# flexcompute/tidy3d

Measured on AMD Instinct MI355X. Metric: Mcells/s on 512^3 Yee grid, higher is better.
Workload: dtype f32; 1 GPU; v0: vacuum, PEC walls, curl stencil only; 512^3 Yee cells, Ez point dipole (GaussianPulse 200 THz), random +-1e-3 initial fields; parallelism=z-slab x1, bytes_per_cell_step=72

## Files before the change

### tidy3d_amd/csrc/fdtd_capi.hip

```cpp
#include <hip/hip_runtime.h>
#include <rccl/rccl.h>

#include <array>
#include <cmath>
#include <cstdarg>
#include <cstdio>
#include <cstdlib>
#include <cstring>
#include <deque>
#include <map>
#include <string>
#include <utility>
#include <algorithm>
#include <vector>

#include "../../include/fdtd_hip.h"
#include "fdtd_kernels.hpp"
#include "fdtd_fused2.hpp"
#include "fdtd_strip.hpp"
#include "fdtd_shell2_host.hpp"
#include "fdtd_aniso.hpp"

using namespace fdtd;

// ... 154 lines not shown
  std::vector<TileClasses> tile_cls;
  int tile_split = -1;
  float2* lut = nullptr;
  int n_media = 0;
  float ca1 = 1.f, cb1 = 0.f;
  std::vector<float> cb_host;
  PmlAxisDev pml[3];
  float *damp_fb[3] = {}, *damp_fc[3] = {};
  int damp_lo[3] = {0, 0, 0}, damp_hi[3] = {0, 0, 0};
  bool has_damp = false;
  std::vector<AdeGroup> ade;
  Disp disp;
  SrcPaged spg;
  std::map<std::array<int, 6>, int> box_paged;
  int spg_on = -1;
  int whatif = 0;
  int disp_on = -1;
  std::vector<AnisoGroup> aniso;
  std::vector<PointSrc> psrc;
  std::vector<Tfsf> tfsf;
  std::vector<Monitor> mons;
  hipStream_t stream = nullptr, comm_stream = nullptr;
  hipEvent_t ev0 = nullptr, ev1 = nullptr;
  std::vector<hipEvent_t> kev;
  std::vector<int> kev_kind;
  double* energy_dev = nullptr;
  int decay_every = 0;
  double shutoff = 0.0;
  long long decay_ref = 0;
  double energy_max = 0.0;
// ... 857 lines not shown
  const MatP mp = mat_params(h);
  DispP dp{nullptr, nullptr, nullptr};
  if (use_disp) dp = DispP{h->disp.dseg, h->disp.cs, h->disp.e1};
  const bool damp = !clip && h->has_damp;
  SrcP sr_used = sr;
  if (h->whatif == 9 && !sr.sseg && !damp && (!use_disp || clip)) {
    SrcPaged& S = h->spg;
    const size_t nseg = (size_t)g.nz * g.ny * ((g.nx + 255) / 256);
    if (!S.sseg && S.state != 1) {
      S.sseg_host.assign(nseg, -1);
      SrcT tab{};
      if (dev_upload(h, &S.sseg, (const int*)S.sseg_host.data(), nseg) || dev_upload(h, &S.tab, &tab, 1)) return -1;
    }
    if (S.sseg && S.state != 1) { sr_used.sseg = S.sseg; sr_used.t = S.tab; }
  }
  const int wv = h->whatif == 19 ? 9 : ((h->whatif >= 1 && h->whatif <= 15 && h->whatif != 9) ? h->whatif : 0);
  const auto word = [&](bool rep) {
    return fused2_opt(h->mem_hints != 0, h->mat4 != nullptr, !(tb->mons.empty() && (!tb->with_sources || h->src_h_nodes == 0) && !tb->dstart),
                      clip != nullptr, damp, use_disp, sr_used.sseg != nullptr, wv, rep, W);
  };
  const bool rep_capable = n_seams > 0 && !clip && (W == 16 || h->seam_defer == 2) && fused2_rep_word(word(false));
  const int opt = word(rep_capable && (h->seam_pending || h->whatif == 17));
  const auto no_sweep = [&] { return fail(h, "launch_fused2: no instantiation of the sweep for opt 0x%x, %d waves", opt, W); };
  if (!fused2_instantiated(fused2_lb(W, opt), opt)) return no_sweep();
  if (sr.sseg) { *sources2_done = true; h->spg.pairs++; }
  float* const rep_arr = h->seam_buf ? h->seam_buf + seam_scratch_floats(g, nbx) : nullptr;
  if (h->seam_pending && !rep_capable) flush_seams(h, st);
  h->seam_pending = false;
  bool defer = defer_ok && rep_capable && h->seam_defer != 0 && h->whatif == 0;
  if (defer) {
    bool e_post = false;
    for (const PointSrc& s : h->psrc) e_post = e_post || (s.n_e && n + 1 < s.n_steps);
    if ((e_post && !*sources2_done) || (h->has_damp && !dmp.e2)) defer = false;
  }
  const int blocks = remap ? ((total + 7) / 8) * 8 : total;
  const FdtdSolver::TileClasses* tc = tile_classes(h, W, zc, box, nbx, nby, nbz, use_disp, sr_used.sseg != nullptr);
  const bool split = tc && (use_disp || sr_used.sseg || (tc->n_bg > 0 && (h->tile_split == 1 || 8 * tc->n_bg >= tc->n_all)));
  const bool launched = launch_fused2_step(Fused2Launch{st, W, opt, blocks, g, h->f, h->f2, sp, mp, zc, nbx, nby, nbz, remap, inj, h->seam_buf, dmp, box,
                                                        TileClassP{split ? tc->dev : nullptr}, dp, sr_used});
  time_end(h, st);
  if (!launched) return no_sweep();
// ... 3080 lines not shown
      h->twostep_w = w;
      h->twostep_zc = zc;
      return 0;
    }
    case FDTD_OPT_PML_SPLIT: h->pml_split = value < 0 ? -1 : (value != 0); return 0;
    case FDTD_OPT_SHELL_PAIRS: h->shell_on = value < 0 ? -1 : value; return 0;
    case FDTD_OPT_STRIP: if (value % 64 < 1 || (value / 64 != 3 && value / 64 != 4)) break; h->strip_zc = value % 64; h->strip_occ = value / 64; return 0;
    case FDTD_OPT_SHELL2: h->shell2_on = value < 0 ? -1 : (value > 3 ? 1 : value); return 0;
    case FDTD_OPT_DEBUG_SYNC: h->debug_sync = value != 0; return 0;
    case FDTD_OPT_TILE_SPLIT: h->tile_split = value < 0 ? -1 : (value != 0); return 0;
    case FDTD_OPT_SRC_PAGED:
      h->spg_on = value < 0 ? -1 : (value != 0);
      if (h->spg.state == -1 && value != 0) h->spg.state = 0;
      return 0;
    case FDTD_OPT_SLAB_BOXES_FIRST: if (value < 0 || value > 3) break; h->slab_boxes_first = value; return 0;
    case FDTD_OPT_WHATIF: if (value < 0 || value > 19) break; h->whatif = value; return 0;
    case FDTD_OPT_SEAM_DEFER: if (value > 2) break; h->seam_defer = value < 0 ? -1 : value; return 0;
    case FDTD_OPT_DISP:
      if (h->disp.state == 1 && value == 0) break;
      h->disp_on = value < 0 ? -1 : (value != 0);
      if (h->disp.state == -1 && value != 0) h->disp.state = 0;
      return 0;
    case FDTD_OPT_SHELL2_SHAPE: {
      if (value <= 0) { h->shell2_qw = 0; h->shell2_ww = 8; h->shell2_zcw = 0; h->shell2_ws = 6; h->shell2_zcs = 0; return 0; }
      const int qw = value % 128, ww = (value >> 7) % 8 + ((value >> 7) % 8 == 0 ? 8 : 0), zcw = (value >> 10) % 128;
      const int ws = (value >> 17) % 16, zcs = (value >> 21) % 128;
      if ((qw != 0 && qw < 3) || qw > 64 || ws > 8) break;
      h->shell2_qw = qw; h->shell2_ww = ww; h->shell2_zcw = zcw;
      h->shell2_ws = ws > 0 ? ws : 6; h->shell2_zcs = zcs;
      return 0;
    }
// ... 45 lines not shown
```

### tidy3d_amd/csrc/fdtd_fused2.hip

```cpp
#include "fdtd_static_kernels.hpp"
#include "fdtd_kernels2.hpp"

namespace fdtd {

void launch_inject_values(hipStream_t st, float* val, const float* w_re, const float* w_im, const float2* wave,
                          long long step, int n) {
  hipLaunchKernelGGL(inject_values_kernel, dim3(1), dim3(256), 0, st, val, w_re, w_im, wave, step, n);
}

static FDTD_F2_LAUNCHER(launch_fused2_step_base, FDTD_F2_LIST_OWN)

bool launch_fused2_step(const Fused2Launch& L) {
  if (L.opt & kF2Src) return launch_fused2_step_src(L);
  if (fused2_whatif(L.opt)) return launch_fused2_step_whatif(L);
  if (L.opt & kF2Disp) return launch_fused2_step_disp(L);
  if (L.opt & kF2Clip) return launch_fused2_step_clip(L);
  return launch_fused2_step_base(L);
}

void launch_inject_table(hipStream_t st, float* tab, long long stride, long long off, const float* w_re, const float* w_im,
                         const float2* wave, long long n_steps, int n) {
  const unsigned blocks = (unsigned)((n_steps * n + 255) / 256);
  hipLaunchKernelGGL(inject_table_kernel, dim3(blocks), dim3(256), 0, st, tab, stride, off, w_re, w_im, wave, n_steps, n);
}

void launch_pair_record(hipStream_t st, const PairRecP& r, long long max_cells, const GridP& g, const FieldP& a, const FieldP& b,
                        const float* cap) {
  const dim3 grid((unsigned)((max_cells + 255) / 256), (unsigned)(r.n_mon * 6));
  hipLaunchKernelGGL(pair_record_kernel, grid, dim3(256), 0, st, r, g, a, b, cap);
}

void launch_dft_record_dump(hipStream_t st, const DftDumpP& r, const float* dump, float2* acc, long long cells, long long fstride,
                            const float2* phase, int nf) {
  const dim3 grid((unsigned)((cells + 255) / 256), (unsigned)r.n);
  hipLaunchKernelGGL(dft_record_dump_kernel, grid, dim3(256), 0, st, r, dump, acc, cells, fstride, phase, nf);
}

void launch_seams(hipStream_t st, const GridP& g, const FieldP& b, const StepP& s, const MatP& m, const float* seam,
                  int n_seams, const DampT& dmp, const ClipP& clip, const InjP& inj, const SrcP& sr, float* rep) {
  const long long nt = (long long)n_seams * (clip.j1 - clip.j0) * (clip.k1 - clip.k0);
  if (nt <= 0) return;
  const unsigned blocks = (unsigned)((nt + 255) / 256);
  hipLaunchKernelGGL(seam_kernel, dim3(blocks), dim3(256), 0, st, g, b, s, m, seam, n_seams, dmp, clip, inj, sr, rep);
}

void launch_seam_flush(hipStream_t st, const GridP& g, const FieldP& b, const float* rep, int n_seams) {
  const long long nt = (long long)n_seams * g.ny * g.nz;
  if (nt <= 0) return;
  hipLaunchKernelGGL(seam_flush_kernel, dim3((unsigned)((nt + 255) / 256)), dim3(256), 0, st, g, b, rep, n_seams);
}

}
```

### tidy3d_amd/csrc/fdtd_fused2.hpp

```cpp
#pragma once
#include "fdtd_kernels.hpp"

namespace fdtd {

constexpr int kMaxInj = 256;
struct InjP {
  int n;
  const int* start;
  const int4* ent;
  const float* val;
  const float* val2;
  int e2_in_sweep;
  float* cap;
  const int* dstart;
  const int* dlist;
  const struct DumpBox* dboxes;
  float* dump;
};
struct DumpBox {
  int lo0, lo1, lo2, nx, ny, nz;
  int off[6];
};
constexpr int kMaxDumps = 8;
struct DampT {
// ... 16 lines not shown
  const float* e1b;
  const float* h2b;
  const float* e2b;
};
struct SrcP {
  const int* sseg = nullptr;
  const SrcT* t = nullptr;
};
constexpr int kF2NT = 1;
constexpr int kF2Mat = 2;
constexpr int kF2Mon = 4;
constexpr int kF2Damp = 8;
constexpr int kF2Clip = 16;
constexpr int kF2Disp = 32;
constexpr int kF2Src = 64;
constexpr int kF2WhatifShift = 8, kF2WhatifMask = 15;
constexpr int kF2NoExj = 4096;
constexpr int kF2Rep = 8192;
constexpr int fused2_whatif(int opt) { return (opt >> kF2WhatifShift) & kF2WhatifMask; }
constexpr int fused2_whatif_word(int wv) { return kF2NT | (wv << kF2WhatifShift); }
constexpr bool fused2_rep_word(int opt) { return (opt & ~(kF2NT | kF2Mat | kF2Damp)) == 0; }

constexpr int fused2_opt(bool nt, bool mat, bool mon, bool clip, bool damp, bool disp, bool src, int whatif, bool rep, int W) {
  int opt = (nt ? kF2NT : 0) | (mat ? kF2Mat : 0) | (mon ? kF2Mon : 0) | (clip ? kF2Clip : (damp ? kF2Damp : 0)) |
            (disp ? kF2Disp | kF2NT : 0) | (src ? kF2Src | kF2Mon | kF2NT : 0);
  if (whatif && opt == kF2NT && (W == 16 || whatif == 13 || whatif == 14)) opt = fused2_whatif_word(whatif);
  return opt | (rep ? kF2Rep : 0);
}
constexpr int fused2_lb(int waves, int opt) {
  if ((opt & kF2Rep) || fused2_whatif(opt)) return 1024;
  if (waves <= 8) return 512;
  return (waves <= 12 && !(opt & (kF2Src | kF2Disp))) ? 768 : 1024;
// ... 9 lines not shown
#define FDTD_F2_LIST_REP(X) FDTD_F2_ANY_MAT(FDTD_F2_AT1024, X, kF2Rep) FDTD_F2_ANY_MAT(FDTD_F2_AT1024, X, kF2Rep | kF2Damp)
#define FDTD_F2_LIST_BASE(X) FDTD_F2_BASE_AT(FDTD_F2_AT512, X) FDTD_F2_BASE_AT(FDTD_F2_AT768, X) FDTD_F2_BASE_AT(FDTD_F2_AT1024, X)
#define FDTD_F2_LIST_CLIP(X) FDTD_F2_ANY_MON(FDTD_F2_AT512, X, kF2Clip) FDTD_F2_ANY_MON(FDTD_F2_AT768, X, kF2Clip) FDTD_F2_ANY_MON(FDTD_F2_AT1024, X, kF2Clip)
#define FDTD_F2_DISP_MON(AT, X, O) AT(X, kF2Disp | kF2Mat | kF2NT | (O)) AT(X, kF2Disp | kF2Mat | kF2NT | kF2Mon | (O))
#define FDTD_F2_DISP_AT(AT, X) FDTD_F2_DISP_MON(AT, X, 0) FDTD_F2_DISP_MON(AT, X, kF2Damp) FDTD_F2_DISP_MON(AT, X, kF2Clip)
#define FDTD_F2_LIST_DISP(X) FDTD_F2_DISP_AT(FDTD_F2_AT512, X) FDTD_F2_DISP_AT(FDTD_F2_AT1024, X)
#define FDTD_F2_SRC_MAT(AT, X, O) AT(X, kF2Src | kF2Mon | kF2NT | (O)) AT(X, kF2Src | kF2Mon | kF2NT | kF2Mat | (O))
#define FDTD_F2_SRC_DISP(AT, X, O) AT(X, kF2Src | kF2Mon | kF2NT | kF2Mat | kF2Disp | (O))
#define FDTD_F2_SRC_AT(AT, X)                                                                          \
  FDTD_F2_SRC_MAT(AT, X, 0) FDTD_F2_SRC_MAT(AT, X, kF2Damp) FDTD_F2_SRC_MAT(AT, X, kF2Clip)              \
  FDTD_F2_SRC_DISP(AT, X, kF2Clip) FDTD_F2_SRC_DISP(AT, X, 0) FDTD_F2_SRC_DISP(AT, X, kF2Damp)
#define FDTD_F2_LIST_SRC(X) FDTD_F2_SRC_AT(FDTD_F2_AT512, X) FDTD_F2_SRC_AT(FDTD_F2_AT1024, X)
#define FDTD_F2_WV(X, WV) X(1024, fused2_whatif_word(WV))
#define FDTD_F2_LIST_WHATIF(X)                                                                                        \
  FDTD_F2_WV(X, 1) FDTD_F2_WV(X, 2) FDTD_F2_WV(X, 3) FDTD_F2_WV(X, 4) FDTD_F2_WV(X, 5) FDTD_F2_WV(X, 6) FDTD_F2_WV(X, 7) FDTD_F2_WV(X, 8) \
  FDTD_F2_WV(X, 9) FDTD_F2_WV(X, 10) FDTD_F2_WV(X, 11) FDTD_F2_WV(X, 12) FDTD_F2_WV(X, 13) FDTD_F2_WV(X, 14) FDTD_F2_WV(X, 15)
#define FDTD_F2_LIST_OWN(X) FDTD_F2_LIST_REP(X) FDTD_F2_LIST_BASE(X)
#define FDTD_F2_LIST_ALL(X) FDTD_F2_LIST_OWN(X) FDTD_F2_LIST_CLIP(X) FDTD_F2_LIST_DISP(X) FDTD_F2_LIST_SRC(X) FDTD_F2_LIST_WHATIF(X)
constexpr int fused2_key(int lb, int opt) { return opt * 2048 + lb; }
constexpr bool fused2_instantiated(int lb, int opt) {
  switch (fused2_key(lb, opt)) {
#define FDTD_F2_X(LBV, OV) case fused2_key(LBV, OV):
    FDTD_F2_LIST_ALL(FDTD_F2_X)
#undef FDTD_F2_X
      return true;
    default: return false;
  }
}
constexpr bool fused2_words_instantiated() {
  for (int W = 4; W <= 16; ++W)
    for (int in = 0; in < 128; ++in) {
      const bool nt = in & 1, mat = in & 2, mon = in & 4, clip = in & 8, damp = in & 16, disp = in & 32, src = in & 64;
      if ((clip && damp) || (disp && !mat)) continue;
      for (int wv = 0; wv <= 15; ++wv) {
        const int opt = fused2_opt(nt, mat, mon, clip, damp, disp, src, wv, false, W);
        if (wv && !fused2_whatif(opt)) continue;
        if (!fused2_instantiated(fused2_lb(W, opt), opt)) return false;
        const int rep = fused2_opt(nt, mat, mon, clip, damp, disp, src, wv, true, W);
        if (!clip && fused2_rep_word(opt) && !fused2_instantiated(fused2_lb(W, rep), rep)) return false;
      }
    }
  return true;
}
static_assert(fused2_words_instantiated(), "fused2_opt forms a word that no list of instantiations holds");

#if !defined(FDTD_NO_EXJ)
#define FDTD_NO_EXJ 0
#endif
constexpr bool fused2_exj(int lb, int opt) { return !FDTD_NO_EXJ && (opt & kF2Damp) == 0 && !(lb == 512 && (opt & kF2Mat) != 0); }
constexpr int fused2_xch_arrays(int lb, int opt) {
  const int wv = fused2_whatif(opt);
  if (wv) return wv == 13 ? 9 : ((wv >= 10 && wv <= 12) ? 6 + (wv == 11 ? 2 : 3) : 8);
  return fused2_exj(lb, opt) ? 9 : 8;
}
constexpr size_t fused2_lds_bytes(int lb, int opt, int waves) {
  return ((size_t)fused2_xch_arrays(lb, opt) * waves * 64 + ((opt & kF2Damp) ? 2 * 64 : 0)) * sizeof(float4) + ((opt & kF2Mat) ? (size_t)kMaxMedia * sizeof(float2) : 0);
}
static_assert(fused2_lds_bytes(1024, kF2NT | kF2Mat | kF2Mon | kF2Clip | kF2Disp | kF2Src, 16) <= 160 * 1024 && fused2_lds_bytes(1024, kF2Mat | kF2Damp, 16) <= 160 * 1024 &&
              2 * fused2_lds_bytes(512, kF2NT, 8) <= 160 * 1024 && 2 * fused2_lds_bytes(512, kF2Mat | kF2Damp, 8) <= 160 * 1024,
              "fused2_step_kernel: LDS of a workgroup (two per CU for eight waves)");
constexpr bool fused2_lds_pinned(int lb, int opt) {
  const int wv = fused2_whatif(opt), w = lb / 64;
  if (wv) return fused2_lds_bytes(lb, opt, 16) == ((size_t)(wv == 13 ? 9 : ((wv >= 10 && wv <= 12) ? 6 + (wv == 11 ? 2 : 3) : 8)) * 16 * 64) * sizeof(float4);
  return fused2_lds_bytes(lb, opt, w) == ((size_t)(fused2_exj(lb, opt) ? 9 : 8) * w * 64 + ((opt & 8) ? 2 * 64 : 0)) * sizeof(float4) + ((opt & 2) ? (size_t)kMaxMedia * sizeof(float2) : 0);
}
#define FDTD_F2_X(LBV, OV) && fused2_lds_pinned(LBV, OV)
static_assert(true FDTD_F2_LIST_ALL(FDTD_F2_X), "fused2_lds_bytes: the LDS of a listed instantiation changed");
#undef FDTD_F2_X
constexpr int kMaxCap = 1024;
constexpr int kSeamArrays = 13;

void launch_inject_values(hipStream_t st, float* val, const float* w_re, const float* w_im, const float2* wave,
                          long long step, int n);
struct Fused2Launch {
  hipStream_t st;
  int waves, opt, grid_blocks;
  GridP g; FieldP a, b; StepP s; MatP m;
  int zchunk, nbx, nby, nbz, xcd_remap;
  InjP inj; float* seam; DampT dmp; ClipP clip; TileClassP tcl; DispP dp; SrcP sr;
// ... 22 lines not shown
  BoxP box[kPairMons];
  int nc[kPairMons];
  int comp[kPairMons][6];
  int cap_off[kPairMons];
  float* out_n[kPairMons];
  float* out_m[kPairMons];
};
void launch_pair_record(hipStream_t st, const PairRecP& r, long long max_cells, const GridP& g, const FieldP& a, const FieldP& b,
                        const float* cap);
struct DftDumpP { int n; int slot[3]; int off[3]; };
void launch_dft_record_dump(hipStream_t st, const DftDumpP& r, const float* dump, float2* acc, long long cells, long long fstride,
                            const float2* phase, int nf);
void launch_seams(hipStream_t st, const GridP& g, const FieldP& b, const StepP& s, const MatP& m, const float* seam,
                  int n_seams, const DampT& dmp, const ClipP& clip, const InjP& inj, const SrcP& sr = SrcP{}, float* rep = nullptr);
constexpr int kRepArraysHost = 7;
inline size_t seam_scratch_floats(const GridP& g, int n_tiles_x) { return (size_t)n_tiles_x * kSeamArrays * (size_t)(g.nz + 2) * (size_t)g.ny; }
inline size_t seam_rep_floats(const GridP& g, int n_tiles_x) { return (size_t)n_tiles_x * kRepArraysHost * (size_t)g.nz * (size_t)g.ny; }
void launch_seam_flush(hipStream_t st, const GridP& g, const FieldP& b, const float* rep, int n_seams);

}
```

### tidy3d_amd/csrc/fdtd_kernels2.hpp

```cpp
#pragma once
#include "fdtd_fused2.hpp"

namespace fdtd {

__global__ __launch_bounds__(256) void pair_record_kernel(PairRecP r, GridP g, FieldP a, FieldP b, const float* cap) {
  const int mi = blockIdx.y / 6, ic = blockIdx.y % 6;
  if (mi >= r.n_mon || ic >= r.nc[mi]) return;
  const BoxP bx = r.box[mi];
  const long long cells = (long long)bx.nx * bx.ny * bx.nz;
  const long long t = (long long)blockIdx.x * blockDim.x + threadIdx.x;
  if (t >= cells) return;
  const int c = r.comp[mi][ic];
  const int lx = (int)(t % bx.nx), ly = (int)((t / bx.nx) % bx.ny), lz = (int)(t / ((long long)bx.nx * bx.ny));
  const long long p = (long long)(bx.lo2 + lz) * g.sxy + (long long)(bx.lo1 + ly) * g.nx + bx.lo0 + lx;
  const long long idx = (long long)ic * cells + t;
  const float* fa = c == 0 ? a.ex : (c == 1 ? a.ey : (c == 2 ? a.ez : (c == 3 ? a.hx : (c == 4 ? a.hy : a.hz))));
  const float* fb = c == 0 ? b.ex : (c == 1 ? b.ey : (c == 2 ? b.ez : (c == 3 ? b.hx : (c == 4 ? b.hy : b.hz))));
  const float mid = cap[r.cap_off[mi] + idx];
  float* on = r.out_n[mi];
  float* om = r.out_m[mi];
  if (c < 3) {
    if (on && !r.pre_done) on[idx] = 1.0f * fa[p];
    if (om) om[idx] = 1.0f * mid;
  } else {
// ... 24 lines not shown
  if (g >= n_steps * n) return;
  const long long step = g / n;
  const int t = (int)(g % n);
  const float2 a = wave[step];
  tab[step * stride + off + t] = w_re[t] * a.x - w_im[t] * a.y;
}

__global__ __launch_bounds__(256) void inject_values_kernel(float* val, const float* w_re, const float* w_im,
                                                            const float2* wave, long long step, int n) {
  const int t = threadIdx.x;
  if (t >= n) return;
  const float2 a = wave[step];
  val[t] = w_re[t] * a.x - w_im[t] * a.y;
}

__device__ __forceinline__ long long seam_at(const GridP& g, int seam, int arr, int j, int k) {
  return (((long long)seam * kSeamArrays + arr) * (g.nz + 2) + (k + 1)) * g.ny + j;
}

constexpr int kRepArrays = 7;
__device__ __forceinline__ long long rep_base(const GridP& g, int n_tiles_x) {
  return (long long)n_tiles_x * kSeamArrays * (g.nz + 2) * g.ny;
}
__device__ __forceinline__ long long rep_at(const GridP& g, int seam, int arr, int j, int k) {
  return (((long long)seam * kRepArrays + arr) * g.nz + k) * g.ny + j;
}

__device__ __forceinline__ float lane_next(float v) {
#if defined(__HIP_DEVICE_COMPILE__)
  const int x = __builtin_bit_cast(int, v);
  return __builtin_bit_cast(float, __builtin_amdgcn_update_dpp(x, x, 0x130, 0xf, 0xf, false));
#else
  return __shfl_down(v, 1);
#endif
}
__device__ __forceinline__ float lane_prev(float v) {
#if defined(__HIP_DEVICE_COMPILE__)
// ... 20 lines not shown
#endif
}
__device__ __forceinline__ void lds_dma_fence() {
#if defined(__HIP_DEVICE_COMPILE__)
  asm volatile("s_waitcnt lgkmcnt(0)" ::: "memory");
#endif
}

__device__ __forceinline__ int opaque_lane(int v) {
#if defined(__HIP_DEVICE_COMPILE__)
  asm volatile("" : "+v"(v));
#endif
  return v;
}

__device__ __forceinline__ int lane_value(int v, int l) {
#if defined(__HIP_DEVICE_COMPILE__)
  return __builtin_amdgcn_readlane(v, l);
#else
  return __shfl(v, l);
#endif
}

template <int LB, int OPT>
__device__ __forceinline__ void fused2_step_tile(const GridP& g, const FieldP& a, const FieldP& b, const StepP& s, const MatP& m,
                                                 int zchunk, int nbx, int nby, int nbz, const InjP& inj,
                                                 float* __restrict__ seam, const DampT& dmp, const ClipP& clip, int t,
                                                 const DispP& dp, const SrcP& sr) {
  constexpr int V = 4;
  constexpr bool SRC = (OPT & kF2Src) != 0;
  constexpr bool NT = (OPT & kF2NT) != 0, MAT = (OPT & kF2Mat) != 0, MON = (OPT & kF2Mon) != 0;
  constexpr bool DISP = (OPT & kF2Disp) != 0;
  constexpr int WHATIF = fused2_whatif(OPT);
  constexpr int PF = (WHATIF >= 10 && WHATIF <= 12) ? WHATIF : 0;
  constexpr bool EZL = WHATIF == 15;
// ... 23 lines not shown
    for (int q = 0; q < NXCH; ++q) xch[q * slot + me] = z4;
  }
  [[maybe_unused]] float4* xdm = xch + (EXJ ? 9 : 8) * slot;
  [[maybe_unused]] float2* lut_s = reinterpret_cast<float2*>(xdm + (DAMP ? 2 * 64 : 0));
  if constexpr (MAT) {
    for (int q = me; q < m.n_media; q += slot) lut_s[q] = m.lut[q];
  }
  if constexpr (DAMP) {
    if (ty == 0) {
      const int ii = (tile_x * 64 + tx) * V;
      float4 b4 = {1.f, 1.f, 1.f, 1.f}, c4 = {1.f, 1.f, 1.f, 1.f};
      if (ii < g.nx) { b4 = *reinterpret_cast<const float4*>(dmp.fb[0] + ii); c4 = *reinterpret_cast<const float4*>(dmp.fc[0] + ii); }
      xdm[tx] = b4; xdm[64 + tx] = c4;
    }
  }
  __syncthreads();
  const float ca = m.ca1, cb = m.cb1;
  const int k0 = (CLIP ? clip.k0 : 0) + tile_z * zchunk;
  const int k1 = min(k0 + zchunk, CLIP ? clip.k1 : g.nz);
  const int kA = k0 > 0 ? k0 - 1 : 0;
  int j = (CLIP ? clip.j0 : 0) + tile_y * R + ty - 2;
  const bool row_ok = (j >= 0) && (j < g.ny);
  if (!row_ok) {
    if constexpr (WHATIF != 6 && WHATIF != 7 && WHATIF != 8)
      for (int k = kA; k <= k1; ++k) { __syncthreads(); if constexpr (WHATIF != 2) __syncthreads(); }
    return;
  }
  const int i0 = (tile_x * 64 + tx) * V;
  const unsigned ux = (unsigned)i0;
  const unsigned ub = ux * 4u;
// ... 82 lines not shown
      const float czp = dmp.fc[2][kA - 1];
      const float4 b4 = xdm[tx], c4 = xdm[64 + tx];
      const float bx[V] = {b4.x, b4.y, b4.z, b4.w}, cx[V] = {c4.x, c4.y, c4.z, c4.w};
#pragma unroll
      for (int e = 0; e < V; ++e) { ho[e] *= bx[e] * cyv * czp; hoy[e] *= cx[e] * byv * czp; }
    }
#pragma unroll
    for (int e = 0; e < V; ++e) h1x[e] = upd_h(ho[e], ch, ezj[e] - ezm[e], ipy, eyk[e] - eym[e], ipz);
#pragma unroll
    for (int e = 0; e < V; ++e) {
      const float ez_ip = (e + 1 < V) ? ezm[(e + 1) % V] : ezx;
      h1y[e] = upd_h(hoy[e], ch, exk[e] - exm[e], ipz, ez_ip - ezm[e], ipx[e]);
    }
  }
  int cur = 0;
  const long long seam_arr = (long long)(g.nz + 2) * g.ny;
  const long long seam_row = seam_at(g, tile_x, 0, j, 0);
  struct Ld {
    float exn[V], eyn[V], ezk[V], exj[V], ezj[V], hxn[V], hyn[V], hzn[V];
    float eyx_g, ezx_g;
    float exn_m, ez_mm, ey_mm, ex_jm, hy_o, hz_o;
  };
  [[maybe_unused]] float4* pfb = xch + NXCH * slot;
  [[maybe_unused]] auto pf_issue = [&](int k) __attribute__((always_inline)) {
    if constexpr (PF != 0) {
      const long long pb = (long long)k * g.sxy + rowb;
      const long long up = (k < g.nz) ? g.sxy : 0;
      lds_dma_fence();
      if constexpr (PF == 10) {
        lds_dma16(uni(a.hx + pb), ubc, pfb + 0 * slot + ty * 64, tx);
        lds_dma16(uni(a.hy + pb), ubc, pfb + 1 * slot + ty * 64, tx);
        lds_dma16(uni(a.hz + pb), ubc, pfb + 2 * slot + ty * 64, tx);
// ... 96 lines not shown
    if constexpr (PF != 0) {
      lds_dma_wait();
      if constexpr (PF == 10) { pf_take(0, L.hxn); pf_take(1, L.hyn); pf_take(2, L.hzn); }
      else if constexpr (PF == 11) { pf_take(0, L.eyn); pf_take(1, L.hyn); }
      else { pf_take(0, L.exn); pf_take(1, L.eyn); pf_take(2, L.ezk); }
    }
  };
  Ld LA, LB2;
  auto body = [&](int k, Ld& L) __attribute__((always_inline)) {
    const int txo = (MAT || DAMP) ? tx : opaque_lane(tx);
    const int i0o = (tile_x * 64 + txo) * V;
    const bool act = i0o < g.nx, last_x = i0o + V >= g.nx, first_x = i0o == 0;
    const bool xh = act && txo == 0 && (!first_x || per_x);
    [[maybe_unused]] const bool wall_x0 = first_x && !pmc_x0 && !per_x;
    const bool seam_l = (txo == 63 && !last_x) || (per_x && last_x), seam_r = txo == 0 && (tile_x > 0 || per_x);
    const long long seam_back = (tile_x > 0 ? -1 : (long long)(nbx - 1)) * kSeamArrays * seam_arr;
    const long long pb = (long long)k * g.sxy + rowb;
    const float ipz = s.ipz[k], idz = s.idz[k];
    [[maybe_unused]] float bzk = 1.f, czk = 1.f;
    if constexpr (DAMP) { bzk = dmp.fb[2][min(k, g.nz - 1)]; czk = dmp.fc[2][min(k, g.nz - 1)]; }
    int q0 = 0, q1 = 0;
    if (inj.n > 0) { q0 = inj.start[k]; q1 = inj.start[k + 1]; }
    [[maybe_unused]] int d0 = 0, d1 = 0;
    if constexpr (MON) { if (inj.dstart) { d0 = inj.dstart[k]; d1 = inj.dstart[k + 1]; } }
    float hy_m = 0.f, hz_m = 0.f;
    float (&exn)[V] = L.exn, (&eyn)[V] = L.eyn, (&ezk)[V] = L.ezk, (&exj)[V] = L.exj, (&ezj)[V] = L.ezj;
    float (&hxn)[V] = L.hxn, (&hyn)[V] = L.hyn, (&hzn)[V] = L.hzn;
    [[maybe_unused]] uint32_t rw = kBgWord;
    if constexpr (MAT) {
      if (do_e1) rw = m.roww[((long long)min(k, g.nz - 1) * g.ny + j) * nbx + tile_x];
    }
// ... 231 lines not shown
                for (int e = 0; e < V; ++e) {
                  const int lx = i0o + e - bx.lo0;
                  if (lx >= 0 && lx < bx.nx && act && (!CLIP || (i0o + e >= clip.i0 && i0o + e < clip.i1))) {
                    if (bx.off[0] >= 0) inj.dump[bx.off[0] + rowo + lx] = e1xn[e];
                    if (bx.off[1] >= 0) inj.dump[bx.off[1] + rowo + lx] = e1yn[e];
                    if (bx.off[2] >= 0) inj.dump[bx.off[2] + rowo + lx] = e1zn[e];
                    if (bx.off[3] >= 0) inj.dump[bx.off[3] + rowo + lx] = hxn[e];
                    if (bx.off[4] >= 0) inj.dump[bx.off[4] + rowo + lx] = hyn[e];
                    if (bx.off[5] >= 0) inj.dump[bx.off[5] + rowo + lx] = hzn[e];
                  }
                }
              }
            }
          }
        }
        if (WHATIF != 9 && (CLIP || (own && k >= k0 && k < k1)) && act) {
          float* sp = seam + seam_row + (long long)k * g.ny;
          if (seam_l) {
            sp[0] = hyn[V - 1];
            sp[seam_arr] = hzn[V - 1];
            sp[2 * seam_arr] = e1xn[V - 1];
            sp[3 * seam_arr] = e1yn[V - 1];
            sp[4 * seam_arr] = e1zn[V - 1];
          }
          if (seam_r) {
            sp[5 * seam_arr + seam_back] = e1yn[0];
            sp[6 * seam_arr + seam_back] = e1zn[0];
          }
        }
      }
    }
    float h2x[V], h2y[V], h2z[V];
    unspecified<V>(h2x); unspecified<V>(h2y); unspecified<V>(h2z);
    if (do_h2 && k > kA) {
      if constexpr (DAMP) {
        {
          const float4 b4 = xdm[tx];
          const float bx[V] = {b4.x, b4.y, b4.z, b4.w};
#pragma unroll
          for (int e = 0; e < V; ++e) h1x[e] *= bx[e] * cyv * cz_m;
        }
        {
// ... 47 lines not shown
        t0 = make_float4(e1x[0], e1x[1], e1x[2], e1x[3]); t1 = make_float4(e1z[0], e1z[1], e1z[2], e1z[3]);
      } else {
        t0 = xch[(4 + (E1S ? 0 : (cur ^ 1) * 2) + 0) * slot + me + 64];
        t1 = xch[(4 + (E1S ? 0 : (cur ^ 1) * 2) + 1) * slot + me + 64];
      }
      const float exj1[V] = {t0.x, t0.y, t0.z, t0.w}, ezj1[V] = {t1.x, t1.y, t1.z, t1.w};
#pragma unroll
      for (int e = 0; e < V; ++e) {
        const float ey_ip = (e + 1 < V) ? e1y[(e + 1) % V] : eyx;
        const float ez_ip = (e + 1 < V) ? e1z[(e + 1) % V] : ezx;
        h2x[e] = upd_h(h1x[e], ch, ezj1[e] - e1z[e], ipy, e1yn[e] - e1y[e], ipz_m);
        h2y[e] = upd_h(h1y[e], ch, e1xn[e] - e1x[e], ipz_m, ez_ip - e1z[e], ipx[e]);
        h2z[e] = upd_h(h1z[e], ch, ey_ip - e1y[e], ipx[e], exj1[e] - e1x[e], ipy);
      }
      if constexpr (CLIP) {
        if (act) {
          float* sq = seam + seam_row + (long long)(k - 1) * g.ny;
          if (seam_l) {
            sq[7 * seam_arr] = h2x[V - 1];
            sq[8 * seam_arr] = h2y[V - 2];
            sq[9 * seam_arr] = h2z[V - 2];
          }
          if (seam_r) {
            sq[10 * seam_arr + seam_back] = h2x[0];
            sq[11 * seam_arr + seam_back] = h2y[0];
            sq[12 * seam_arr + seam_back] = h2z[0];
          }
        }
      }
    }
    if constexpr (WHATIF != 6) {
      float4 t4;
      if constexpr (!E1S) {
        t4.x = e1xn[0]; t4.y = e1xn[1]; t4.z = e1xn[2]; t4.w = e1xn[3];
        xch[(4 + cur * 2 + 0) * slot + me] = t4;
        t4.x = e1zn[0]; t4.y = e1zn[1]; t4.z = e1zn[2]; t4.w = e1zn[3];
        xch[(4 + cur * 2 + 1) * slot + me] = t4;
      }
      if constexpr (EXJ) {
        t4.x = exn[0]; t4.y = exn[1]; t4.z = exn[2]; t4.w = exn[3];
        xch[XE * slot + me] = t4;
// ... 112 lines not shown
        if (dmp.e2) {
          {
            const float4 c4 = xdm[64 + tx];
            const float cx[V] = {c4.x, c4.y, c4.z, c4.w};
#pragma unroll
            for (int e = 0; e < V; ++e) ex[e] *= cx[e] * byv * bz_m;
          }
          {
            const float4 b4 = xdm[tx];
            const float bx[V] = {b4.x, b4.y, b4.z, b4.w};
#pragma unroll
            for (int e = 0; e < V; ++e) { ey[e] *= bx[e] * cyv * bz_m; ez[e] *= bx[e] * byv * cz_m; }
          }
        }
      }
      if (act && (!CLIP || (i0o >= clip.i0 && i0o < clip.i1))) {
        float* sq = seam + seam_row + (long long)(k - 1) * g.ny;
        if (!CLIP && WHATIF != 9 && txo == 63 && !last_x) {
          sq[7 * seam_arr] = h2x[V - 1];
          sq[8 * seam_arr] = h2y[V - 2];
          sq[9 * seam_arr] = h2z[V - 2];
        }
        if (!CLIP && WHATIF != 9 && txo == 0 && tile_x > 0) {
          sq[10 * seam_arr - kSeamArrays * seam_arr] = h2x[0];
          sq[11 * seam_arr - kSeamArrays * seam_arr] = h2y[0];
          sq[12 * seam_arr - kSeamArrays * seam_arr] = h2z[0];
        }
        const long long po = pb - g.sxy + i0;
        if (WHATIF != 5 || ex[0] == 3.0e38f) {
          stv_h<V, NT>(b.hx + po, h2x);
          stv_h<V, NT>(b.hy + po, h2y);
          stv_h<V, NT>(b.hz + po, h2z);
          stv_h<V, NT>(b.ex + po, ex);
          stv_h<V, NT>(b.ey + po, ey);
          stv_h<V, NT>(b.ez + po, ez);
        }
      }
    }
#pragma unroll
    for (int e = 0; e < V; ++e) {
      h2xm[e] = h2x[e]; h2ym[e] = h2y[e];
      h1x[e] = hxn[e]; h1y[e] = hyn[e]; h1z[e] = hzn[e];
      e1x[e] = e1xn[e]; e1y[e] = e1yn[e]; e1z[e] = e1zn[e];
      exk[e] = exn[e]; eyk[e] = eyn[e];
    }
    exk_m = L.exn_m;
    ipz_m = ipz; idz_m = idz;
    qm0 = q0; qm1 = q1;
    if constexpr (DAMP) { bz_m = bzk; cz_m = czk; }
    if constexpr (MAT) rw_m = rw;
    if constexpr (SRC) ss_m = ss;
// ... 48 lines not shown
  }
  constexpr int OPTK = OPT | (fused2_exj(LB, OPT) ? 0 : kF2NoExj);
  if constexpr ((OPT & kF2Src) != 0) {
    if (tcl.cls && !(tcl.cls[t] & 4)) {
      fused2_tile_by_class<LB, (OPTK & ~kF2Src)>(g, a, b, s, m, zchunk, nbx, nby, nbz, inj, seam, dmp, clip, t, dp, sr, tcl);
      return;
    }
  }
  fused2_tile_by_class<LB, OPTK>(g, a, b, s, m, zchunk, nbx, nby, nbz, inj, seam, dmp, clip, t, dp, sr, tcl);
}

__global__ __launch_bounds__(256) void seam_kernel(GridP g, FieldP b, StepP s, MatP m,
                                                   const float* __restrict__ seam, int n_seams, DampT dmp, ClipP clip, InjP inj, SrcP sr,
                                                   float* __restrict__ rep) {
  const long long t = (long long)blockIdx.x * blockDim.x + threadIdx.x;
  const int nj = clip.j1 - clip.j0;
  const long long per = (long long)nj * (clip.k1 - clip.k0);
  if (t >= per * n_seams) return;
  const int sm = (int)(t / per);
  const int k = clip.k0 + (int)((t % per) / nj), j = clip.j0 + (int)(t % nj);
  const bool wrap = g.bcx0 == BC_PERIODIC && sm == n_seams - 1;
  const int c = wrap ? g.nx : (sm + 1) * 256;
  const int cc = wrap ? 0 : c;
  const bool wl = c - 1 >= clip.i0 && c - 1 < clip.i1, wr = cc >= clip.i0 && cc < clip.i1;
  if (!wl && !wr) return;
  const float ch = g.ch;
  const float ipx = s.ipx[c - 1];
  auto A = [&](int a, int jj, int kk) { return seam[seam_at(g, sm, a, jj, kk)]; };
  auto h2 = [&](int jj, int kk, float& hy, float& hz) {
    const float e1x = A(2, jj, kk), e1y = A(3, jj, kk), e1z = A(4, jj, kk);
    const float e1x_jp = (jj + 1 < g.ny) ? A(2, jj + 1, kk) : 0.f;
    float h1y = A(0, jj, kk), h1z = A(1, jj, kk);
    if (dmp.fb[0]) {
      const float cxv = dmp.fc[0][c - 1];
      h1y *= cxv * dmp.fb[1][jj] * dmp.fc[2][kk];
// ... 99 lines not shown
```

Baseline: 199,900 Mcells/s.

## Stage seam writes in LDS and flush blocked z-contiguous seam scratch layout

Re-lays out the x-seam scratch buffer so each (seam, j) row stores blocks of 8 consecutive z planes with one slot per array, instead of separate arrays strided by ny. The fused kernel now stages per-plane seam values in LDS and flushes each 8-plane block with one coalesced wave store, rather than issuing scattered single-float global stores every plane. The seam kernel is remapped to 64-lane tiles over (j-block, z-block). The old path is kept as whatif 16. In exchange it adds LDS per wave, wave barriers and extra flush logic.

```diff
diff --git a/tidy3d_amd/csrc/fdtd_capi.hip b/tidy3d_amd/csrc/fdtd_capi.hip
--- a/tidy3d_amd/csrc/fdtd_capi.hip
+++ b/tidy3d_amd/csrc/fdtd_capi.hip
@@ -192,6 +192,7 @@
   SrcPaged spg;
   std::map<std::array<int, 6>, int> box_paged;
   int spg_on = -1;
+  bool seam_scratch_dirty = false;
   int whatif = 0;
   int disp_on = -1;
   std::vector<AnisoGroup> aniso;
@@ -1079,7 +1080,7 @@
     }
     if (S.sseg && S.state != 1) { sr_used.sseg = S.sseg; sr_used.t = S.tab; }
   }
-  const int wv = h->whatif == 19 ? 9 : ((h->whatif >= 1 && h->whatif <= 15 && h->whatif != 9) ? h->whatif : 0);
+  const int wv = h->whatif == 19 ? 9 : (h->whatif == 20 ? 16 : ((h->whatif >= 1 && h->whatif <= 15 && h->whatif != 9) ? h->whatif : 0));
   const auto word = [&](bool rep) {
     return fused2_opt(h->mem_hints != 0, h->mat4 != nullptr, !(tb->mons.empty() && (!tb->with_sources || h->src_h_nodes == 0) && !tb->dstart),
                       clip != nullptr, damp, use_disp, sr_used.sseg != nullptr, wv, rep, W);
@@ -1090,6 +1091,11 @@
   if (!fused2_instantiated(fused2_lb(W, opt), opt)) return no_sweep();
   if (sr.sseg) { *sources2_done = true; h->spg.pairs++; }
   float* const rep_arr = h->seam_buf ? h->seam_buf + seam_scratch_floats(g, nbx) : nullptr;
+  if (h->seam_buf && h->seam_scratch_dirty && fused2_whatif(opt) != 16) {
+    hipMemsetAsync(h->seam_buf, 0, seam_scratch_floats(g, nbx) * sizeof(float), st);
+    h->seam_scratch_dirty = false;
+  }
+  if (fused2_whatif(opt) == 16) h->seam_scratch_dirty = true;
   if (h->seam_pending && !rep_capable) flush_seams(h, st);
   h->seam_pending = false;
   bool defer = defer_ok && rep_capable && h->seam_defer != 0 && h->whatif == 0;
@@ -4200,7 +4206,7 @@
       if (h->spg.state == -1 && value != 0) h->spg.state = 0;
       return 0;
     case FDTD_OPT_SLAB_BOXES_FIRST: if (value < 0 || value > 3) break; h->slab_boxes_first = value; return 0;
-    case FDTD_OPT_WHATIF: if (value < 0 || value > 19) break; h->whatif = value; return 0;
+    case FDTD_OPT_WHATIF: if (value < 0 || value > 20) break; h->whatif = value; return 0;
     case FDTD_OPT_SEAM_DEFER: if (value > 2) break; h->seam_defer = value < 0 ? -1 : value; return 0;
     case FDTD_OPT_DISP:
       if (h->disp.state == 1 && value == 0) break;
diff --git a/tidy3d_amd/csrc/fdtd_fused2.hip b/tidy3d_amd/csrc/fdtd_fused2.hip
--- a/tidy3d_amd/csrc/fdtd_fused2.hip
+++ b/tidy3d_amd/csrc/fdtd_fused2.hip
@@ -38,7 +38,9 @@
 
 void launch_seams(hipStream_t st, const GridP& g, const FieldP& b, const StepP& s, const MatP& m, const float* seam,
                   int n_seams, const DampT& dmp, const ClipP& clip, const InjP& inj, const SrcP& sr, float* rep) {
-  const long long nt = (long long)n_seams * (clip.j1 - clip.j0) * (clip.k1 - clip.k0);
+  if (clip.j1 <= clip.j0 || clip.k1 <= clip.k0) return;
+  const long long nzb = clip.k1 / kSeamP - (clip.k0 + 1) / kSeamP + 1, njb = (clip.j1 - clip.j0 + 7) / 8;
+  const long long nt = (long long)n_seams * njb * nzb * 64;
   if (nt <= 0) return;
   const unsigned blocks = (unsigned)((nt + 255) / 256);
   hipLaunchKernelGGL(seam_kernel, dim3(blocks), dim3(256), 0, st, g, b, s, m, seam, n_seams, dmp, clip, inj, sr, rep);
diff --git a/tidy3d_amd/csrc/fdtd_fused2.hpp b/tidy3d_amd/csrc/fdtd_fused2.hpp
--- a/tidy3d_amd/csrc/fdtd_fused2.hpp
+++ b/tidy3d_amd/csrc/fdtd_fused2.hpp
@@ -54,8 +54,8 @@
 constexpr int kF2Clip = 16;
 constexpr int kF2Disp = 32;
 constexpr int kF2Src = 64;
-constexpr int kF2WhatifShift = 8, kF2WhatifMask = 15;
-constexpr int kF2NoExj = 4096;
+constexpr int kF2WhatifShift = 8, kF2WhatifMask = 31;
+constexpr int kF2NoExj = 16384;
 constexpr int kF2Rep = 8192;
 constexpr int fused2_whatif(int opt) { return (opt >> kF2WhatifShift) & kF2WhatifMask; }
 constexpr int fused2_whatif_word(int wv) { return kF2NT | (wv << kF2WhatifShift); }
@@ -95,7 +95,8 @@
 #define FDTD_F2_WV(X, WV) X(1024, fused2_whatif_word(WV))
 #define FDTD_F2_LIST_WHATIF(X)                                                                                        \
   FDTD_F2_WV(X, 1) FDTD_F2_WV(X, 2) FDTD_F2_WV(X, 3) FDTD_F2_WV(X, 4) FDTD_F2_WV(X, 5) FDTD_F2_WV(X, 6) FDTD_F2_WV(X, 7) FDTD_F2_WV(X, 8) \
-  FDTD_F2_WV(X, 9) FDTD_F2_WV(X, 10) FDTD_F2_WV(X, 11) FDTD_F2_WV(X, 12) FDTD_F2_WV(X, 13) FDTD_F2_WV(X, 14) FDTD_F2_WV(X, 15)
+  FDTD_F2_WV(X, 9) FDTD_F2_WV(X, 10) FDTD_F2_WV(X, 11) FDTD_F2_WV(X, 12) FDTD_F2_WV(X, 13) FDTD_F2_WV(X, 14) FDTD_F2_WV(X, 15) \
+  FDTD_F2_WV(X, 16)
 #define FDTD_F2_LIST_OWN(X) FDTD_F2_LIST_REP(X) FDTD_F2_LIST_BASE(X)
 #define FDTD_F2_LIST_ALL(X) FDTD_F2_LIST_OWN(X) FDTD_F2_LIST_CLIP(X) FDTD_F2_LIST_DISP(X) FDTD_F2_LIST_SRC(X) FDTD_F2_LIST_WHATIF(X)
 constexpr int fused2_key(int lb, int opt) { return opt * 2048 + lb; }
@@ -113,7 +114,7 @@
     for (int in = 0; in < 128; ++in) {
       const bool nt = in & 1, mat = in & 2, mon = in & 4, clip = in & 8, damp = in & 16, disp = in & 32, src = in & 64;
       if ((clip && damp) || (disp && !mat)) continue;
-      for (int wv = 0; wv <= 15; ++wv) {
+      for (int wv = 0; wv <= 16; ++wv) {
         const int opt = fused2_opt(nt, mat, mon, clip, damp, disp, src, wv, false, W);
         if (wv && !fused2_whatif(opt)) continue;
         if (!fused2_instantiated(fused2_lb(W, opt), opt)) return false;
@@ -134,16 +135,19 @@
   if (wv) return wv == 13 ? 9 : ((wv >= 10 && wv <= 12) ? 6 + (wv == 11 ? 2 : 3) : 8);
   return fused2_exj(lb, opt) ? 9 : 8;
 }
+constexpr int kSeamP = 8;
+constexpr int kSeamStageFloats = 13 * kSeamP;
 constexpr size_t fused2_lds_bytes(int lb, int opt, int waves) {
-  return ((size_t)fused2_xch_arrays(lb, opt) * waves * 64 + ((opt & kF2Damp) ? 2 * 64 : 0)) * sizeof(float4) + ((opt & kF2Mat) ? (size_t)kMaxMedia * sizeof(float2) : 0);
+  return ((size_t)fused2_xch_arrays(lb, opt) * waves * 64 + ((opt & kF2Damp) ? 2 * 64 : 0)) * sizeof(float4) + ((opt & kF2Mat) ? (size_t)kMaxMedia * sizeof(float2) : 0) +
+         (size_t)waves * kSeamStageFloats * sizeof(float);
 }
 static_assert(fused2_lds_bytes(1024, kF2NT | kF2Mat | kF2Mon | kF2Clip | kF2Disp | kF2Src, 16) <= 160 * 1024 && fused2_lds_bytes(1024, kF2Mat | kF2Damp, 16) <= 160 * 1024 &&
               2 * fused2_lds_bytes(512, kF2NT, 8) <= 160 * 1024 && 2 * fused2_lds_bytes(512, kF2Mat | kF2Damp, 8) <= 160 * 1024,
               "fused2_step_kernel: LDS of a workgroup (two per CU for eight waves)");
 constexpr bool fused2_lds_pinned(int lb, int opt) {
   const int wv = fused2_whatif(opt), w = lb / 64;
-  if (wv) return fused2_lds_bytes(lb, opt, 16) == ((size_t)(wv == 13 ? 9 : ((wv >= 10 && wv <= 12) ? 6 + (wv == 11 ? 2 : 3) : 8)) * 16 * 64) * sizeof(float4);
-  return fused2_lds_bytes(lb, opt, w) == ((size_t)(fused2_exj(lb, opt) ? 9 : 8) * w * 64 + ((opt & 8) ? 2 * 64 : 0)) * sizeof(float4) + ((opt & 2) ? (size_t)kMaxMedia * sizeof(float2) : 0);
+  if (wv) return fused2_lds_bytes(lb, opt, 16) == ((size_t)(wv == 13 ? 9 : ((wv >= 10 && wv <= 12) ? 6 + (wv == 11 ? 2 : 3) : 8)) * 16 * 64) * sizeof(float4) + 16 * 416;
+  return fused2_lds_bytes(lb, opt, w) == ((size_t)(fused2_exj(lb, opt) ? 9 : 8) * w * 64 + ((opt & 8) ? 2 * 64 : 0)) * sizeof(float4) + ((opt & 2) ? (size_t)kMaxMedia * sizeof(float2) : 0) + (size_t)w * 416;
 }
 #define FDTD_F2_X(LBV, OV) && fused2_lds_pinned(LBV, OV)
 static_assert(true FDTD_F2_LIST_ALL(FDTD_F2_X), "fused2_lds_bytes: the LDS of a listed instantiation changed");
@@ -196,7 +200,10 @@
 void launch_seams(hipStream_t st, const GridP& g, const FieldP& b, const StepP& s, const MatP& m, const float* seam,
                   int n_seams, const DampT& dmp, const ClipP& clip, const InjP& inj, const SrcP& sr = SrcP{}, float* rep = nullptr);
 constexpr int kRepArraysHost = 7;
-inline size_t seam_scratch_floats(const GridP& g, int n_tiles_x) { return (size_t)n_tiles_x * kSeamArrays * (size_t)(g.nz + 2) * (size_t)g.ny; }
+constexpr int kSeamSlots = 16;
+static_assert(kSeamStageFloats == kSeamArrays * kSeamP && kSeamArrays + 1 <= kSeamSlots, "seam staging: one slot per scratch array and plane of a block");
+constexpr int seam_blocks(int nz) { return (nz + 2 + kSeamP - 1) / kSeamP; }
+inline size_t seam_scratch_floats(const GridP& g, int n_tiles_x) { return (size_t)n_tiles_x * (size_t)g.ny * (size_t)seam_blocks(g.nz) * kSeamSlots * kSeamP; }
 inline size_t seam_rep_floats(const GridP& g, int n_tiles_x) { return (size_t)n_tiles_x * kRepArraysHost * (size_t)g.nz * (size_t)g.ny; }
 void launch_seam_flush(hipStream_t st, const GridP& g, const FieldP& b, const float* rep, int n_seams);
 
diff --git a/tidy3d_amd/csrc/fdtd_kernels2.hpp b/tidy3d_amd/csrc/fdtd_kernels2.hpp
--- a/tidy3d_amd/csrc/fdtd_kernels2.hpp
+++ b/tidy3d_amd/csrc/fdtd_kernels2.hpp
@@ -62,13 +62,14 @@
   val[t] = w_re[t] * a.x - w_im[t] * a.y;
 }
 
+__device__ __forceinline__ int seam_slot(int arr) { return arr < 7 ? arr : arr + 1; }
 __device__ __forceinline__ long long seam_at(const GridP& g, int seam, int arr, int j, int k) {
-  return (((long long)seam * kSeamArrays + arr) * (g.nz + 2) + (k + 1)) * g.ny + j;
+  return ((((long long)seam * g.ny + j) * seam_blocks(g.nz) + ((k + 1) / kSeamP)) * kSeamSlots + seam_slot(arr)) * kSeamP + (k + 1) % kSeamP;
 }
 
 constexpr int kRepArrays = 7;
 __device__ __forceinline__ long long rep_base(const GridP& g, int n_tiles_x) {
-  return (long long)n_tiles_x * kSeamArrays * (g.nz + 2) * g.ny;
+  return (long long)n_tiles_x * g.ny * seam_blocks(g.nz) * (kSeamSlots * kSeamP);
 }
 __device__ __forceinline__ long long rep_at(const GridP& g, int seam, int arr, int j, int k) {
   return (((long long)seam * kRepArrays + arr) * g.nz + k) * g.ny + j;
@@ -119,11 +120,28 @@
   return v;
 }
 
+__device__ __forceinline__ int opaque_uniform(int v) {
+#if defined(__HIP_DEVICE_COMPILE__)
+  asm volatile("" : "+s"(v));
+#endif
+  return v;
+}
+
 __device__ __forceinline__ int lane_value(int v, int l) {
 #if defined(__HIP_DEVICE_COMPILE__)
   return __builtin_amdgcn_readlane(v, l);
 #else
   return __shfl(v, l);
+#endif
+}
+
+__device__ __forceinline__ void wave_sync() {
+#if defined(__HIP_DEVICE_COMPILE__)
+  __builtin_amdgcn_fence(__ATOMIC_RELEASE, "wavefront");
+  __builtin_amdgcn_wave_barrier();
+  __builtin_amdgcn_fence(__ATOMIC_ACQUIRE, "wavefront");
+#else
+  (void)__ballot(1);
 #endif
 }
 
@@ -177,6 +195,8 @@
       xdm[tx] = b4; xdm[64 + tx] = c4;
     }
   }
+  constexpr int NARR = PF ? NXCH + NPF : (EZL ? 8 : (EXJ ? 9 : 8));
+  [[maybe_unused]] const int stg_off = (NARR * slot + (DAMP ? 2 * 64 : 0)) * 4 + (MAT ? 2 * kMaxMedia : 0) + ty * kSeamStageFloats;
   __syncthreads();
   const float ca = m.ca1, cb = m.cb1;
   const int k0 = (CLIP ? clip.k0 : 0) + tile_z * zchunk;
@@ -289,8 +309,24 @@
     }
   }
   int cur = 0;
-  const long long seam_arr = (long long)(g.nz + 2) * g.ny;
-  const long long seam_row = seam_at(g, tile_x, 0, j, 0);
+  const long long seam_tile = (long long)g.ny * seam_blocks(g.nz) * (kSeamSlots * kSeamP);
+  const long long seam_row = seam_at(g, tile_x, 0, j, -1);
+  const bool stage_l = (tile_x * 256 + 256 < g.nx) || per_x, stage_r = tile_x > 0 || per_x;
+  [[maybe_unused]] auto stage_flush = [&](int group, int kf, int kl) __attribute__((always_inline)) {
+    wave_sync();
+    const int ln = opaque_lane(tx);
+    const float* stg = reinterpret_cast<const float*>(xch) + opaque_uniform(stg_off);
+    const int zi = kl + 1, zb = zi & ~(kSeamP - 1);
+    const int z = zb + (ln & (kSeamP - 1));
+    const int nl = (group ? 3 : 5) * kSeamP, na = (group ? 6 : 7) * kSeamP;
+    const float v = stg[(group ? 7 * kSeamP : 0) + (ln < na ? ln : 0)];
+    const bool in = z > kf && z <= zi;
+    float* sp = seam + seam_row + (long long)zb * kSeamSlots + (group ? 8 * kSeamP : 0);
+    if (stage_l && in && ln < nl) *at(uni(sp), (unsigned)ln * 4u) = v;
+    if (stage_r && in && ln >= nl && ln < na) *at(uni(sp + (tile_x > 0 ? -1 : (long long)(nbx - 1)) * seam_tile), (unsigned)ln * 4u) = v;
+  };
+  [[maybe_unused]] const long long old_arr = (long long)(g.nz + 2) * g.ny;
+  [[maybe_unused]] const long long old_row = (((long long)tile_x * kSeamArrays) * (g.nz + 2) + 1) * g.ny + j;
   struct Ld {
     float exn[V], eyn[V], ezk[V], exj[V], ezj[V], hxn[V], hyn[V], hzn[V];
     float eyx_g, ezx_g;
@@ -417,7 +453,6 @@
     const bool xh = act && txo == 0 && (!first_x || per_x);
     [[maybe_unused]] const bool wall_x0 = first_x && !pmc_x0 && !per_x;
     const bool seam_l = (txo == 63 && !last_x) || (per_x && last_x), seam_r = txo == 0 && (tile_x > 0 || per_x);
-    const long long seam_back = (tile_x > 0 ? -1 : (long long)(nbx - 1)) * kSeamArrays * seam_arr;
     const long long pb = (long long)k * g.sxy + rowb;
     const float ipz = s.ipz[k], idz = s.idz[k];
     [[maybe_unused]] float bzk = 1.f, czk = 1.f;
@@ -679,18 +714,35 @@
             }
           }
         }
-        if (WHATIF != 9 && (CLIP || (own && k >= k0 && k < k1)) && act) {
-          float* sp = seam + seam_row + (long long)k * g.ny;
-          if (seam_l) {
-            sp[0] = hyn[V - 1];
-            sp[seam_arr] = hzn[V - 1];
-            sp[2 * seam_arr] = e1xn[V - 1];
-            sp[3 * seam_arr] = e1yn[V - 1];
-            sp[4 * seam_arr] = e1zn[V - 1];
-          }
-          if (seam_r) {
-            sp[5 * seam_arr + seam_back] = e1yn[0];
-            sp[6 * seam_arr + seam_back] = e1zn[0];
+        if constexpr (WHATIF == 16) {
+          if (own && k >= k0 && k < k1 && act) {
+            float* sp = seam + old_row + (long long)k * g.ny;
+            if (seam_l) {
+              sp[0] = hyn[V - 1];
+              sp[old_arr] = hzn[V - 1];
+              sp[2 * old_arr] = e1xn[V - 1];
+              sp[3 * old_arr] = e1yn[V - 1];
+              sp[4 * old_arr] = e1zn[V - 1];
+            }
+            if (seam_r) {
+              sp[(5 - kSeamArrays) * old_arr] = e1yn[0];
+              sp[(6 - kSeamArrays) * old_arr] = e1zn[0];
+            }
+          }
+        } else if (WHATIF != 9 && (CLIP || (own && k >= k0 && k < k1))) {
+          float* stg = reinterpret_cast<float*>(xch) + opaque_uniform(stg_off) + ((k + 1) & (kSeamP - 1));
+          if (act) {
+            if (seam_l) {
+              stg[0 * kSeamP] = hyn[V - 1];
+              stg[1 * kSeamP] = hzn[V - 1];
+              stg[2 * kSeamP] = e1xn[V - 1];
+              stg[3 * kSeamP] = e1yn[V - 1];
+              stg[4 * kSeamP] = e1zn[V - 1];
+            }
+            if (seam_r) {
+              stg[5 * kSeamP] = e1yn[0];
+              stg[6 * kSeamP] = e1zn[0];
+            }
           }
         }
       }
@@ -768,17 +820,17 @@
         h2z[e] = upd_h(h1z[e], ch, ey_ip - e1y[e], ipx[e], exj1[e] - e1x[e], ipy);
       }
       if constexpr (CLIP) {
+        float* stg = reinterpret_cast<float*>(xch) + opaque_uniform(stg_off) + (k & (kSeamP - 1));
         if (act) {
-          float* sq = seam + seam_row + (long long)(k - 1) * g.ny;
           if (seam_l) {
-            sq[7 * seam_arr] = h2x[V - 1];
-            sq[8 * seam_arr] = h2y[V - 2];
-            sq[9 * seam_arr] = h2z[V - 2];
+            stg[7 * kSeamP] = h2x[V - 1];
+            stg[8 * kSeamP] = h2y[V - 2];
+            stg[9 * kSeamP] = h2z[V - 2];
           }
           if (seam_r) {
-            sq[10 * seam_arr + seam_back] = h2x[0];
-            sq[11 * seam_arr + seam_back] = h2y[0];
-            sq[12 * seam_arr + seam_back] = h2z[0];
+            stg[10 * kSeamP] = h2x[0];
+            stg[11 * kSeamP] = h2y[0];
+            stg[12 * kSeamP] = h2z[0];
           }
         }
       }
@@ -921,18 +973,36 @@
           }
         }
       }
+      if constexpr (WHATIF == 16) {
+        if (act) {
+          float* sq = seam + old_row + (long long)(k - 1) * g.ny;
+          if (txo == 63 && !last_x) {
+            sq[7 * old_arr] = h2x[V - 1];
+            sq[8 * old_arr] = h2y[V - 2];
+            sq[9 * old_arr] = h2z[V - 2];
+          }
+          if (txo == 0 && tile_x > 0) {
+            sq[(10 - kSeamArrays) * old_arr] = h2x[0];
+            sq[(11 - kSeamArrays) * old_arr] = h2y[0];
+            sq[(12 - kSeamArrays) * old_arr] = h2z[0];
+          }
+        }
+      } else if constexpr (!CLIP && WHATIF != 9) {
+        float* stg = reinterpret_cast<float*>(xch) + opaque_uniform(stg_off) + (k & (kSeamP - 1));
+        if (act) {
+          if (txo == 63 && !last_x) {
+            stg[7 * kSeamP] = h2x[V - 1];
+            stg[8 * kSeamP] = h2y[V - 2];
+            stg[9 * kSeamP] = h2z[V - 2];
+          }
+          if (txo == 0 && tile_x > 0) {
+            stg[10 * kSeamP] = h2x[0];
+            stg[11 * kSeamP] = h2y[0];
+            stg[12 * kSeamP] = h2z[0];
+          }
+        }
+      }
       if (act && (!CLIP || (i0o >= clip.i0 && i0o < clip.i1))) {
-        float* sq = seam + seam_row + (long long)(k - 1) * g.ny;
-        if (!CLIP && WHATIF != 9 && txo == 63 && !last_x) {
-          sq[7 * seam_arr] = h2x[V - 1];
-          sq[8 * seam_arr] = h2y[V - 2];
-          sq[9 * seam_arr] = h2z[V - 2];
-        }
-        if (!CLIP && WHATIF != 9 && txo == 0 && tile_x > 0) {
-          sq[10 * seam_arr - kSeamArrays * seam_arr] = h2x[0];
-          sq[11 * seam_arr - kSeamArrays * seam_arr] = h2y[0];
-          sq[12 * seam_arr - kSeamArrays * seam_arr] = h2z[0];
-        }
         const long long po = pb - g.sxy + i0;
         if (WHATIF != 5 || ex[0] == 3.0e38f) {
           stv_h<V, NT>(b.hx + po, h2x);
@@ -942,6 +1012,14 @@
           stv_h<V, NT>(b.ey + po, ey);
           stv_h<V, NT>(b.ez + po, ez);
         }
+      }
+    }
+    if constexpr (WHATIF != 9 && WHATIF != 16) {
+      if (CLIP ? do_e1 : (own && k >= k0 && k < k1)) {
+        if (((k + 1) & (kSeamP - 1)) == kSeamP - 1 || k == (CLIP ? k1 : k1 - 1)) stage_flush(0, CLIP ? kA : k0, k);
+      }
+      if (CLIP ? (do_h2 && k > kA) : (own && k > k0)) {
+        if ((k & (kSeamP - 1)) == kSeamP - 1 || k == k1) stage_flush(1, CLIP ? kA : k0, k - 1);
       }
     }
 #pragma unroll
@@ -1020,11 +1098,13 @@
                                                    const float* __restrict__ seam, int n_seams, DampT dmp, ClipP clip, InjP inj, SrcP sr,
                                                    float* __restrict__ rep) {
   const long long t = (long long)blockIdx.x * blockDim.x + threadIdx.x;
-  const int nj = clip.j1 - clip.j0;
-  const long long per = (long long)nj * (clip.k1 - clip.k0);
-  if (t >= per * n_seams) return;
-  const int sm = (int)(t / per);
-  const int k = clip.k0 + (int)((t % per) / nj), j = clip.j0 + (int)(t % nj);
+  const int zb0 = (clip.k0 + 1) / kSeamP, nzb = clip.k1 / kSeamP - zb0 + 1, njb = (clip.j1 - clip.j0 + 7) / 8;
+  const long long per = (long long)njb * nzb;
+  const long long tile = t >> 6;
+  if (tile >= per * n_seams) return;
+  const int sm = (int)(tile / per), ln = (int)(t & 63);
+  const int k = (zb0 + (int)(tile % nzb)) * kSeamP + (ln & (kSeamP - 1)) - 1, j = clip.j0 + (int)((tile % per) / nzb) * 8 + (ln >> 3);
+  if (k < clip.k0 || k >= clip.k1 || j >= clip.j1) return;
   const bool wrap = g.bcx0 == BC_PERIODIC && sm == n_seams - 1;
   const int c = wrap ? g.nx : (sm + 1) * 256;
   const int cc = wrap ? 0 : c;
```

New measurement: 191,500 Mcells/s. -4.2%, worse.
